# TeamOfProfGuo/Few_Shot_Seg_CWT

Measured on AMD Instinct MI355X. Metric: episodes/sec (473x473, 1-shot, R50) at 1/2/4/8 MI355X; mIoU vs ref, higher is better.
Workload: dtype fp32 (conv stack at fp32 width on the bf16 MFMA: every fp32 operand split exactly into bf16 hi + mid + lo, the six products >= 2^-24 |a||b| summed in fp32; inner loop, CWT, classifier fp32); 1 GPU; CWT inference episode (validate_transformer, batch_size_val=1): PASCAL split-0 1-shot ResNet-50 PSPNet 473x473, adapt_iter 200, heads 4; image_size=473, shot=1, layers=50

## Files before the change

### few_shot_seg_cwt_amd/csrc/conv_body.h

```cpp
#pragma once
#include "common.h"
#include "kernels.h"

namespace cwt {

typedef __bf16 bf16x8 __attribute__((ext_vector_type(8)));

#define CWT_LDS __attribute__((address_space(3)))
#define CWT_GLB __attribute__((address_space(1)))

__device__ __forceinline__ void glds16(const void* src, char* lds_dst) {
  __builtin_amdgcn_global_load_lds((const CWT_GLB void*)src, (CWT_LDS void*)lds_dst, 16, 0, 0);
}

template <int N>
__device__ __forceinline__ void wait_vmcnt() {
  asm volatile("s_waitcnt vmcnt(%0)" ::"n"(N) : "memory");
}

template <int LPT>
__device__ __forceinline__ void wait_tiles(int n) {
  if (n <= 0)
    wait_vmcnt<0>();
  else if (n == 1)
    wait_vmcnt<LPT>();
  else if (n == 2)
    wait_vmcnt<2 * LPT>();
  else if (n == 3)
    wait_vmcnt<3 * LPT>();
  else if (n == 4)
    wait_vmcnt<4 * LPT>();
  else
    wait_vmcnt<5 * LPT>();
}

__device__ __forceinline__ void block_sync_lds() {
  asm volatile("s_waitcnt lgkmcnt(0)" ::: "memory");
  __builtin_amdgcn_s_barrier();
  asm volatile("" ::: "memory");
}

struct Res8 {
  f32x4 a, b;
};
template <int PREC>
__device__ __forceinline__ Res8 load_res8(const ConvSArgs& a, int m, int co) {
  Res8 r;
  if (a.res) {
    const f32x4* rp = (const f32x4*)(a.res + (long)m * a.res_ld + co);
    r.a = rp[0];
    r.b = rp[1];
  } else if (a.res_s) {
    if (PREC == 1) {
      r.a = *(const f32x4*)(a.res_s + (long)m * a.Co + co);
      r.b = f32x4{0.f, 0.f, 0.f, 0.f};
    } else {
      const __bf16* rp = a.res_s + ((long)m * (a.Co >> 5) + (co >> 5)) * 64 + (co & 31);
      r.a = *(const f32x4*)rp;
      r.b = *(const f32x4*)(rp + 32);
    }
  } else {
    r.a = r.b = f32x4{0.f, 0.f, 0.f, 0.f};
  }
  return r;
}

template <int PREC>
__device__ __forceinline__ void store_out8(const ConvSArgs& a, int m, int co, const float* v, const float* sc,
                                           const float* sh, const Res8& rs) {
  float o[8];
#pragma unroll
  for (int i = 0; i < 8; ++i) o[i] = fmaf(v[i], sc[i], sh[i]);
  if (a.res) {
#pragma unroll
    for (int i = 0; i < 4; ++i) {
      o[i] += rs.a[i];
      o[4 + i] += rs.b[i];
    }
  } else if (a.res_s) {
    const bf16x8 rh = __builtin_bit_cast(bf16x8, rs.a), rl = __builtin_bit_cast(bf16x8, rs.b);
#pragma unroll
    for (int i = 0; i < 8; ++i) o[i] += PREC == 1 ? (float)rh[i] : (float)rh[i] + (float)rl[i];
  }
  if (a.relu) {
#pragma unroll
    for (int i = 0; i < 8; ++i) o[i] = fmaxf(o[i], 0.f);
  }
  if (a.y) {
    f32x4* yp = (f32x4*)(a.y + (long)m * a.y_ld + a.y_off + co);
    yp[0] = f32x4{o[0], o[1], o[2], o[3]};
    yp[1] = f32x4{o[4], o[5], o[6], o[7]};
  }
  if (a.ys) {
    bf16x8 hi, lo;
#pragma unroll
    for (int i = 0; i < 8; ++i) {
      hi[i] = (__bf16)o[i];
      lo[i] = (__bf16)(o[i] - (float)hi[i]);
    }
    if (PREC == 1) {
      *(bf16x8*)(a.ys + (long)m * a.Co + co) = hi;
    } else {
      __bf16* sp = a.ys + ((long)m * (a.Co >> 5) + (co >> 5)) * 64 + (co & 31);
      *(bf16x8*)sp = hi;
      *(bf16x8*)(sp + 32) = lo;
    }
  }
}

__device__ __forceinline__ void split3_bf16(const f32x4& x0, const f32x4& x1, bf16x8& h, bf16x8& m, bf16x8& l) {
#pragma unroll
  for (int i = 0; i < 8; ++i) {
    const float v = i < 4 ? x0[i] : x1[i - 4];
    const __bf16 hv = (__bf16)v;
    const float r = v - (float)hv;
    const __bf16 mv = (__bf16)r;
    h[i] = hv;
    m[i] = mv;
    l[i] = (__bf16)(r - (float)mv);
  }
}

template <int BM, int BN, int WAVES_M, int WAVES_N, int NSTG, int PREC, int PF>
__device__ __forceinline__ void conv_s_body(const ConvSArgs& a) {
  static_assert(PREC == 0 || PREC == 1 || PREC == 3 || PREC == 6,
                "PREC: 3 = bf16x3 over the S-layout, 1 = plain bf16, 0 = exact fp32 (f32 MFMA), "
                "6 = fp32 operands split three ways in registers (bf16x6)");
  constexpr int NW = WAVES_M * WAVES_N;
  constexpr int WM = BM / WAVES_M, WN = BN / WAVES_N;
  constexpr int FM = WM / 16, FN = WN / 16;
  constexpr int LA = BM / (8 * NW), LB = BN / (8 * NW);
  constexpr int NLO = PREC == 6 ? BN / 16 : 0;
  constexpr int LBL = PREC == 6 ? (NLO + NW - 1) / NW : 0;
  constexpr int LPT = LA + LB + LBL;
  constexpr int LO_OFF = (BM + BN) * 128;
  constexpr int STG_BYTES = (BM + BN) * 128 + (PREC == 6 ? BN * 64 : 0);
  static_assert(LA * 8 * NW == BM && LB * 8 * NW == BN, "tile rows must split into 8-row pieces per wave");
  static_assert(NSTG >= 2 && NSTG <= 6, "ring depth");
  constexpr int EP_ROWS = WM < 32 ? WM : 32;
  constexpr int EP_LD = WN + 4;
  constexpr int EP_BYTES = NW * EP_ROWS * EP_LD * 4;
  constexpr int SMEM = NSTG * STG_BYTES > EP_BYTES ? NSTG * STG_BYTES : EP_BYTES;
  __shared__ __attribute__((aligned(16))) char smem[SMEM];

  const int tid = threadIdx.x;
  const int lane = tid & 63;
  const int wv = __builtin_amdgcn_readfirstlane(tid >> 6);
  const int wm = wv / WAVES_N, wn = wv % WAVES_N;
  int mt, nt, ks;
  conv_tile_coords(mt, nt, ks);
  const bool batched = PREC == 6 && a.batch > 1;
  const int bidx = batched ? ks : 0;
  if (batched) ks = 0;
  const char* xs_b = (const char*)a.xs + (batched ? bidx * a.xs_bstride : 0L);
  const __bf16* ws_b = a.ws + (batched ? bidx * a.ws_bstride : 0L);
  const __bf16* wl_b = a.ws_lo + (batched ? bidx * a.wl_bstride : 0L);
  float* part_b = a.part + (batched ? (long)bidx * a.M * a.Co : 0L);
  const int m0 = mt * BM, n0 = nt * BN;
  const int kt_begin = ks * a.kt_per_split;
  const int kt_end = min(a.ktiles, kt_begin + a.kt_per_split);
  const int T = kt_end - kt_begin;
  if constexpr ((PF & 64) != 0) {
    asm volatile("" ::"s"(T));
    return;
  }


  const int lrow = lane >> 3, lslot = lane & 7;
  const int cblocks = a.Ci >> (PREC == 1 ? 6 : 5);
  int a_ih0[LA], a_iw0[LA], a_pix0[LA], a_ch[LA];
  const int HoWo = a.Ho * a.Wo;
#pragma unroll
  for (int j = 0; j < LA; ++j) {
    const int r = (wv * LA + j) * 8 + lrow;
    a_ch[j] = (lslot ^ ((r >> 1) & 7)) * 8;
    const int m = m0 + r;
    if (m < a.M) {
      const int n = m / HoWo;
      const int rem = m - n * HoWo;
      const int oh = rem / a.Wo;
      const int ow = rem - oh * a.Wo;
      a_ih0[j] = oh * a.stride - a.pad;
      a_iw0[j] = ow * a.stride - a.pad;
      a_pix0[j] = (n * a.Hi + a_ih0[j]) * a.Wi + a_iw0[j];
    } else {
      a_ih0[j] = -(1 << 28);
      a_iw0[j] = 0;
      a_pix0[j] = 0;
    }
  }
  const int b_rowlen = a.ktiles_total * 64;
  int b_off[LB];
#pragma unroll
  for (int j = 0; j < LB; ++j) {
    const int r = (wv * LB + j) * 8 + lrow;
    b_off[j] = (n0 + r) * b_rowlen + (lslot ^ ((r >> 1) & 7)) * 8;
  }

  int i_cb, i_ky, i_kx;
  {
    const int taps = a.kh * a.kw;
    i_cb = kt_begin / taps;
    const int tap = kt_begin - i_cb * taps;
    i_ky = tap / a.kw;
    i_kx = tap - i_ky * a.kw;
  }
  int i_kt = kt_begin;
  constexpr bool DUAL = (PF & 128) != 0;
  static_assert(!DUAL || (PREC == 6 && (PF & 8) != 0), "dual A source: x6 with buffer addressing");
  __amdgpu_buffer_rsrc_t rsA, rsB, rsL, rsA2;
  int a_roff[LA], b_voff[LB], l_voff[LBL > 0 ? LBL : 1], a_roff2[DUAL ? LA : 1];
#if defined(__HIP_DEVICE_COMPILE__)
  if constexpr (DUAL) {
    const int cbl2 = a.Ci2 >> 5;
    rsA2 = __builtin_amdgcn_make_buffer_rsrc((void*)a.xs2, (short)0, (int)((long)a.N * a.Hi2 * a.Wi2 * cbl2 * 128),
                                             0x00020000);
#pragma unroll
    for (int j = 0; j < LA; ++j) {
      const int m = m0 + (wv * LA + j) * 8 + lrow;
      const int n = m / HoWo, rem = m - n * HoWo;
      const int oh = rem / a.Wo, ow = rem - oh * a.Wo;
      const int pix2 = (n * a.Hi2 + oh * a.stride2) * a.Wi2 + ow * a.stride2;
      a_roff2[j] = m < a.M ? (pix2 * cbl2 * 64 + a_ch[j]) * 2 : (int)0x80000000;
    }
  }
  if constexpr ((PF & 8) != 0) {
    const int cbl = a.Ci >> (PREC == 1 ? 6 : 5);
    const long a_bytes = (long)a.N * a.Hi * a.Wi * cbl * 128;
    rsA = __builtin_amdgcn_make_buffer_rsrc((void*)xs_b, (short)0, (int)a_bytes, 0x00020000);
    rsB = __builtin_amdgcn_make_buffer_rsrc((void*)ws_b, (short)0, (int)((long)a.Co * a.ktiles_total * 128), 0x00020000);
#pragma unroll
    for (int j = 0; j < LA; ++j) a_roff[j] = (a_pix0[j] * cbl * 64 + a_ch[j]) * 2;
#pragma unroll
    for (int j = 0; j < LB; ++j) b_voff[j] = b_off[j] * 2;
    if constexpr (PREC == 6) {
      rsL = __builtin_amdgcn_make_buffer_rsrc((void*)wl_b, (short)0, (int)((long)a.Co * a.ktiles_total * 64),
                                              0x00020000);
#pragma unroll
      for (int j = 0; j < LBL; ++j) {
        const int q = (wv * LBL + j) % NLO;
        const int r = q * 16 + (lane >> 2);
        l_voff[j] = (n0 + r) * a.ktiles_total * 64 + (((lane & 3) ^ ((r >> 2) & 3)) << 4);
      }
    }
  }
#endif
  auto issue = [&](int stg) {
    if (PF & 4) return;
    char* sb = smem + stg * STG_BYTES;
#if defined(__HIP_DEVICE_COMPILE__)
    if constexpr ((PF & 8) != 0) {
      const int dy = i_ky * a.dil, dx = i_kx * a.dil;
      const int uni = ((dy * a.Wi + dx) * cblocks + i_cb) * 128;
      bool second = false;
      if constexpr (DUAL) {
        second = i_kt >= a.kt_switch;
        if (second) {
          const unsigned uni2 = (unsigned)(i_kt - a.kt_switch) * 128u;
#pragma unroll
          for (int j = 0; j < LA; ++j)
            __builtin_amdgcn_raw_ptr_buffer_load_lds(rsA2, (CWT_LDS void*)(sb + (wv * LA + j) * 1024), 16,
                                                     (int)((unsigned)a_roff2[j] + uni2), 0, 0, 0);
        }
      }
      if (!second) {
#pragma unroll
        for (int j = 0; j < LA; ++j) {
          const int ih = a_ih0[j] + dy, iw = a_iw0[j] + dx;
          const bool in = (unsigned)ih < (unsigned)a.Hi && (unsigned)iw < (unsigned)a.Wi;
          __builtin_amdgcn_raw_ptr_buffer_load_lds(rsA, (CWT_LDS void*)(sb + (wv * LA + j) * 1024), 16,
                                                   in ? a_roff[j] + uni : (int)0x80000000, 0, 0, 0);
        }
      }
#pragma unroll
      for (int j = 0; j < LB; ++j)
        __builtin_amdgcn_raw_ptr_buffer_load_lds(rsB, (CWT_LDS void*)(sb + BM * 128 + (wv * LB + j) * 1024), 16,
                                                 b_voff[j], i_kt * 128, 0, 0);
      if constexpr (PREC == 6) {
#pragma unroll
        for (int j = 0; j < LBL; ++j)
          __builtin_amdgcn_raw_ptr_buffer_load_lds(rsL, (CWT_LDS void*)(sb + LO_OFF + ((wv * LBL + j) % NLO) * 1024), 16,
                                                   l_voff[j], i_kt * 64, 0, 0);
      }
      ++i_kt;
      if (++i_kx == a.kw) {
        i_kx = 0;
        if (++i_ky == a.kh) {
          i_ky = 0;
          ++i_cb;
        }
      }
      return;
    }
#endif
    const int dy = i_ky * a.dil, dx = i_kx * a.dil;
    const int shift = dy * a.Wi + dx;
#pragma unroll
    for (int j = 0; j < LA; ++j) {
      const int ih = a_ih0[j] + dy, iw = a_iw0[j] + dx;
      const bool in = (unsigned)ih < (unsigned)a.Hi && (unsigned)iw < (unsigned)a.Wi;
      const __bf16* src = in ? a.xs + ((a_pix0[j] + shift) * cblocks + i_cb) * 64 + a_ch[j] : a.zero;
      glds16(src, sb + (wv * LA + j) * 1024);
    }
#pragma unroll
    for (int j = 0; j < LB; ++j) glds16(a.ws + b_off[j] + i_kt * 64, sb + BM * 128 + (wv * LB + j) * 1024);
    ++i_kt;
    if (++i_kx == a.kw) {
      i_kx = 0;
      if (++i_ky == a.kh) {
        i_ky = 0;
        ++i_cb;
      }
    }
  };

  f32x4 acc[FM][FN];
#pragma unroll
  for (int i = 0; i < FM; ++i)
#pragma unroll
    for (int j = 0; j < FN; ++j) acc[i][j] = f32x4{0.f, 0.f, 0.f, 0.f};

  const int fr = lane & 15, fk = lane >> 4;
  const int swz = (fr >> 1) & 7;
  const int off_hi = fr * 128 + ((fk ^ swz) << 4);
  const int off_lo = fr * 128 + (((4 + fk) ^ swz) << 4);
  const int off_a0 = PREC == 6 ? fr * 128 + (((2 * fk) ^ swz) << 4) : off_hi;
  const int off_a1 = PREC == 6 ? fr * 128 + (((2 * fk + 1) ^ swz) << 4) : off_lo;
  const int off_l = fr * 64 + ((fk ^ ((fr >> 2) & 3)) << 4);
  const int a_row0 = wm * WM, b_row0 = BM + wn * WN;

  constexpr bool LAZY_B = PREC == 6 && (PF & 3) == 0 && FN >= 8;
  struct Frags {
    bf16x8 ah[FM], al[FM], bh[LAZY_B ? 1 : FN], bl[LAZY_B ? 1 : FN];
    bf16x8 bo[PREC == 6 && !LAZY_B ? FN : 1];
  };
  auto read_frags = [&](Frags& F, int stg) {
    const char* sb = smem + stg * STG_BYTES;
#pragma unroll
    for (int j = 0; j < (LAZY_B ? 0 : FN); ++j) {
      const char* p = sb + (b_row0 + j * 16) * 128;
      F.bh[j] = *(const bf16x8*)(p + off_hi);
      F.bl[j] = *(const bf16x8*)(p + off_lo);
    }
#pragma unroll
    for (int i = 0; i < FM; ++i) {
      const char* p = sb + (a_row0 + i * 16) * 128;
      F.ah[i] = *(const bf16x8*)(p + off_a0);
      F.al[i] = *(const bf16x8*)(p + off_a1);
    }
    if constexpr (PREC == 6 && !LAZY_B) {
#pragma unroll
      for (int j = 0; j < FN; ++j) F.bo[j] = *(const bf16x8*)(sb + LO_OFF + (wn * WN + j * 16) * 64 + off_l);
    }
  };
  auto mfmas = [&](const Frags& F, int stg) {
    if (PF & 2) {
#pragma unroll
      for (int i = 0; i < FM; ++i) asm volatile("" ::"v"(F.ah[i]), "v"(F.al[i]));
#pragma unroll
      for (int j = 0; j < (LAZY_B ? 1 : FN); ++j)
        asm volatile("" ::"v"(F.bh[j]), "v"(F.bl[j]), "v"(F.bo[j < (PREC == 6 && !LAZY_B ? FN : 1) ? j : 0]));
      return;
    }
    if constexpr (LAZY_B) {
      const char* sb = smem + stg * STG_BYTES;
      bf16x8 as[FM][3];
#pragma unroll
      for (int i = 0; i < FM; ++i)
        if constexpr ((PF & 16) != 0) {
          as[i][0] = F.ah[i];
          as[i][1] = F.al[i];
          as[i][2] = F.ah[i];
        } else {
          split3_bf16(__builtin_bit_cast(f32x4, F.ah[i]), __builtin_bit_cast(f32x4, F.al[i]), as[i][0], as[i][1],
                      as[i][2]);
        }
#pragma unroll
      for (int j = 0; j < FN; ++j) {
        const char* p = sb + (b_row0 + j * 16) * 128;
        const bf16x8 bh = *(const bf16x8*)(p + off_hi), bm = *(const bf16x8*)(p + off_lo);
        const bf16x8 bl = *(const bf16x8*)(sb + LO_OFF + (wn * WN + j * 16) * 64 + off_l);
#pragma unroll
        for (int i = 0; i < FM; ++i) {
          acc[i][j] = __builtin_amdgcn_mfma_f32_16x16x32_bf16(as[i][1], bm, acc[i][j], 0, 0, 0);
          acc[i][j] = __builtin_amdgcn_mfma_f32_16x16x32_bf16(as[i][2], bh, acc[i][j], 0, 0, 0);
          acc[i][j] = __builtin_amdgcn_mfma_f32_16x16x32_bf16(as[i][0], bl, acc[i][j], 0, 0, 0);
          acc[i][j] = __builtin_amdgcn_mfma_f32_16x16x32_bf16(as[i][1], bh, acc[i][j], 0, 0, 0);
          acc[i][j] = __builtin_amdgcn_mfma_f32_16x16x32_bf16(as[i][0], bm, acc[i][j], 0, 0, 0);
          acc[i][j] = __builtin_amdgcn_mfma_f32_16x16x32_bf16(as[i][0], bh, acc[i][j], 0, 0, 0);
        }
      }
    } else if constexpr (PREC == 6) {
#pragma unroll
      for (int i = 0; i < FM; ++i) {
        bf16x8 ah, am, al;
        split3_bf16(__builtin_bit_cast(f32x4, F.ah[i]), __builtin_bit_cast(f32x4, F.al[i]), ah, am, al);
#pragma unroll
        for (int j = 0; j < FN; ++j) {
          acc[i][j] = __builtin_amdgcn_mfma_f32_16x16x32_bf16(am, F.bl[j], acc[i][j], 0, 0, 0);
          acc[i][j] = __builtin_amdgcn_mfma_f32_16x16x32_bf16(al, F.bh[j], acc[i][j], 0, 0, 0);
          acc[i][j] = __builtin_amdgcn_mfma_f32_16x16x32_bf16(ah, F.bo[j], acc[i][j], 0, 0, 0);
          acc[i][j] = __builtin_amdgcn_mfma_f32_16x16x32_bf16(am, F.bh[j], acc[i][j], 0, 0, 0);
          acc[i][j] = __builtin_amdgcn_mfma_f32_16x16x32_bf16(ah, F.bl[j], acc[i][j], 0, 0, 0);
          acc[i][j] = __builtin_amdgcn_mfma_f32_16x16x32_bf16(ah, F.bh[j], acc[i][j], 0, 0, 0);
        }
      }
    } else {
#pragma unroll
    for (int i = 0; i < FM; ++i)
#pragma unroll
      for (int j = 0; j < FN; ++j) {
        if (PREC == 0) {
          const f32x4 a0 = __builtin_bit_cast(f32x4, F.ah[i]), a1 = __builtin_bit_cast(f32x4, F.al[i]);
          const f32x4 b0 = __builtin_bit_cast(f32x4, F.bh[j]), b1 = __builtin_bit_cast(f32x4, F.bl[j]);
#pragma unroll
          for (int s = 0; s < 4; ++s) acc[i][j] = __builtin_amdgcn_mfma_f32_16x16x4f32(a0[s], b0[s], acc[i][j], 0, 0, 0);
#pragma unroll
          for (int s = 0; s < 4; ++s) acc[i][j] = __builtin_amdgcn_mfma_f32_16x16x4f32(a1[s], b1[s], acc[i][j], 0, 0, 0);
        } else if (PREC == 1) {
          acc[i][j] = __builtin_amdgcn_mfma_f32_16x16x32_bf16(F.ah[i], F.bh[j], acc[i][j], 0, 0, 0);
          acc[i][j] = __builtin_amdgcn_mfma_f32_16x16x32_bf16(F.al[i], F.bl[j], acc[i][j], 0, 0, 0);
        } else {
          acc[i][j] = __builtin_amdgcn_mfma_f32_16x16x32_bf16(F.al[i], F.bh[j], acc[i][j], 0, 0, 0);
          acc[i][j] = __builtin_amdgcn_mfma_f32_16x16x32_bf16(F.ah[i], F.bl[j], acc[i][j], 0, 0, 0);
          acc[i][j] = __builtin_amdgcn_mfma_f32_16x16x32_bf16(F.ah[i], F.bh[j], acc[i][j], 0, 0, 0);
        }
      }
    }
  };

  if constexpr ((PF & 1) == 0) {
#pragma unroll
    for (int s = 0; s < NSTG - 1; ++s)
      if (s < T) issue(s);

    for (int t = 0; t < T; ++t) {
      wait_tiles<LPT>(min(NSTG - 2, T - 1 - t));
      block_sync_lds();
      if (t + NSTG - 1 < T) issue((t + NSTG - 1) % NSTG);
      Frags F;
      read_frags(F, t % NSTG);
      mfmas(F, t % NSTG);
    }
  } else {
#pragma unroll
    for (int s = 0; s < NSTG; ++s)
      if (s < T) issue(s);
    Frags F0, F1;
    if (T > 0) {
      wait_tiles<LPT>(min(NSTG - 1, T - 1));
      block_sync_lds();
      read_frags(F0, 0);
    }
    auto step = [&](int t, Frags& cur, Frags& nxt) {
      if (t + 1 < T) {
        wait_tiles<LPT>(min(T - t - 2, NSTG - 2));
        block_sync_lds();
        if (t + NSTG < T) issue(t % NSTG);
        read_frags(nxt, (t + 1) % NSTG);
      }
      mfmas(cur, -1);
    };
    for (int t = 0; t < T; t += 2) {
      step(t, F0, F1);
      if (t + 1 < T) step(t + 1, F1, F0);
    }
  }

  wait_vmcnt<0>();
  if constexpr ((PF & 32) != 0) {
#pragma unroll
    for (int i = 0; i < FM; ++i)
#pragma unroll
      for (int j = 0; j < FN; ++j) asm volatile("" ::"v"(acc[i][j]));
    return;
  }
  block_sync_lds();
  float* ep = (float*)smem + wv * (EP_ROWS * EP_LD);
  constexpr int LPR = WN / 8;
  constexpr int RPR = 64 / LPR;
  static_assert(LPR * 8 == WN && RPR * LPR == 64 && EP_ROWS % RPR == 0, "epilogue geometry");
  const int er = lane / LPR, eg = lane - er * LPR;
  const int co = n0 + wn * WN + eg * 8;
  float sc[8], sh[8];
#pragma unroll
  for (int i = 0; i < 8; ++i) {
    sc[i] = a.part ? 1.f : a.scale[co + i];
    sh[i] = a.part ? 0.f : a.shift[co + i];
  }
  const int fq = lane >> 4;
  constexpr int NPASS = WM / EP_ROWS, RR = EP_ROWS / RPR;
  const int mrow = m0 + wm * WM + er;
  Res8 resb[2][RR];
  const bool fused = !a.part;
#pragma unroll
  for (int rr = 0; rr < RR; ++rr)
    if (fused) resb[0][rr] = load_res8<PREC>(a, min(mrow + rr * RPR, a.M - 1), co);
#pragma unroll
  for (int pass = 0; pass < NPASS; ++pass) {
#pragma unroll
    for (int fi = 0; fi < EP_ROWS / 16; ++fi)
#pragma unroll
      for (int j = 0; j < FN; ++j)
#pragma unroll
        for (int q = 0; q < 4; ++q) ep[(fi * 16 + fq * 4 + q) * EP_LD + j * 16 + fr] = acc[pass * (EP_ROWS / 16) + fi][j][q];
    asm volatile("s_waitcnt lgkmcnt(0)" ::: "memory");
    f32x4 v0[RR], v1[RR];
#pragma unroll
    for (int rr = 0; rr < RR; ++rr) {
      const int r = rr * RPR + er;
      v0[rr] = *(const f32x4*)(ep + r * EP_LD + eg * 8);
      v1[rr] = *(const f32x4*)(ep + r * EP_LD + eg * 8 + 4);
    }
    if (pass + 1 < NPASS && fused) {
#pragma unroll
      for (int rr = 0; rr < RR; ++rr)
        resb[(pass + 1) & 1][rr] = load_res8<PREC>(a, min(mrow + (pass + 1) * EP_ROWS + rr * RPR, a.M - 1), co);
    }
#pragma unroll
    for (int rr = 0; rr < RR; ++rr) {
      const int m = mrow + pass * EP_ROWS + rr * RPR;
      if (m < a.M) {
        if (!fused) {
          f32x4* pp = (f32x4*)(part_b + ((long)ks * a.M + m) * a.Co + co);
          pp[0] = v0[rr];
          pp[1] = v1[rr];
        } else {
          const float v[8] = {v0[rr][0], v0[rr][1], v0[rr][2], v0[rr][3], v1[rr][0], v1[rr][1], v1[rr][2], v1[rr][3]};
          store_out8<PREC>(a, m, co, v, sc, sh, resb[pass & 1][rr]);
        }
      }
    }
    asm volatile("s_waitcnt lgkmcnt(0)" ::: "memory");
  }
}

ConvPlan plan_heuristic_s(int M, int Co, int ktiles);
void launch_tiles_x6(int stage, const ConvSArgs& a, const ConvPlan& p, dim3 grid, hipStream_t st);
}
```

### few_shot_seg_cwt_amd/csrc/conv_forms.h

```cpp
#pragma once
#include <type_traits>

#include "kernels.h"

namespace cwt {

#define CWT_CONV_FORMS(X, A)                                                                   \
  X(256, 256, 0, 2, 4, 2, 0, 0) A(256, 256, 1, 0) A(256, 256, 2, 0)                            \
  X(256, 128, 0, 4, 2, 3, 0, 0) X(256, 128, 1, 4, 2, 3, 1, 0) A(256, 128, 2, 1)                \
  X(128, 256, 0, 2, 4, 3, 0, 0) X(128, 256, 1, 2, 4, 3, 1, 0) A(128, 256, 2, 1)                \
  X(128, 128, 0, 2, 2, 3, 0, 0) X(128, 128, 1, 2, 2, 3, 1, 0) X(128, 128, 2, 2, 4, 3, 1, 0)    \
  X(128, 128, 4, 2, 2, 2, 0, 0)                                                                \
  X(128, 64, 0, 2, 2, 3, 0, 0) X(128, 64, 1, 2, 2, 3, 1, 0) X(128, 64, 2, 4, 2, 3, 1, 0)       \
  X(64, 128, 0, 2, 2, 3, 0, 0) X(64, 128, 1, 2, 2, 3, 1, 0) X(64, 128, 2, 2, 4, 3, 1, 0)       \
  X(64, 64, 0, 2, 2, 4, 0, 0) X(64, 64, 1, 2, 2, 4, 1, 0) X(64, 64, 2, 2, 4, 4, 1, 0)          \
         \
  X(64, 64, 8, 2, 2, 4, 2, 1) X(64, 64, 9, 2, 2, 4, 4, 1)                                      \
                                             \
  X(128, 128, 10, 2, 4, 3, 3, 1) X(128, 128, 11, 2, 4, 3, 5, 1)

#define CWT_CONV_FORMS_X6(X, A)                                                                \
  X(256, 256, 3, 4, 2, 2, 0, 0) X(256, 128, 3, 8, 1, 2, 0, 0) X(128, 256, 3, 4, 2, 2, 0, 0)    \
  X(128, 128, 3, 4, 1, 3, 0, 0) X(128, 128, 5, 4, 1, 2, 0, 0)                                  \
  X(128, 64, 3, 4, 1, 3, 0, 0) X(128, 64, 5, 4, 1, 2, 0, 0)                                    \
  X(64, 128, 3, 4, 1, 3, 0, 0) X(64, 128, 5, 4, 1, 2, 0, 0)                                    \
  X(64, 64, 3, 4, 1, 4, 0, 0)                                                                  \
    \
      \
                                           \
  X(128, 128, 12, 4, 1, 2, 16, 0) X(128, 128, 14, 4, 1, 2, 4, 0) X(128, 128, 15, 4, 1, 2, 2, 0) \
  X(128, 128, 16, 4, 1, 2, 6, 0) X(128, 128, 17, 4, 1, 2, 38, 0) X(128, 128, 18, 4, 1, 2, 64, 0) \
                                                \
  X(256, 256, 13, 4, 2, 2, 16, 0)                                                              \
    \
    \
  X(128, 128, 24, 2, 2, 2, 128, 0) X(128, 128, 25, 4, 1, 2, 128, 0)                            \
  X(128, 64, 25, 4, 1, 2, 128, 0) X(64, 128, 25, 4, 1, 2, 128, 0)

constexpr int kConvDualVar = 20;

struct ConvForm {
  int bm, bn, var, waves_m, waves_n, nstg, pf;
  bool fixed_tile;
  int alias;
};
const ConvForm* find_conv_form(int prec, int bm, int bn, int var);
const ConvForm* fixed_tile_form(int prec, int var);

template <int LAST, class F>
void with_stage(int stage, F&& f) {
  if constexpr (LAST > 0)
    if (stage >= 0 && stage < LAST) return with_stage<LAST - 1>(stage, f);
  f(std::integral_constant<int, LAST>{});
}

template <class Fam, int STAGE>
void launch_form(const ConvPlan& p, const ConvSArgs& a, dim3 grid, hipStream_t st) {
#define CWT_ROW(BM, BN, VAR, WM, WN, NS, PF, FIXED)     \
  if (p.bm == BM && p.bn == BN && p.var == VAR)         \
    return Fam::template launch<BM, BN, WM, WN, NS, (FIXED && Fam::kStudyStage0) ? 0 : STAGE, PF>(a, grid, st);
#define CWT_ALIAS(BM, BN, VAR, TARGET)
  CWT_CONV_FORMS(CWT_ROW, CWT_ALIAS)
  if constexpr (Fam::kX6) {
    CWT_CONV_FORMS_X6(CWT_ROW, CWT_ALIAS)
  }
#undef CWT_ROW
#undef CWT_ALIAS
}

#define CWT_CONV_FAMILY(NAME, KERNEL, X6, STUDY_STAGE0)                                        \
  struct NAME {                                                                                \
    static constexpr bool kX6 = X6, kStudyStage0 = STUDY_STAGE0;                               \
    template <int BM, int BN, int WM, int WN, int NS, int STAGE, int PF>                       \
    static void launch(const ConvSArgs& a, dim3 grid, hipStream_t st) {                        \
      hipLaunchKernelGGL((KERNEL<BM, BN, WM, WN, NS, STAGE, PF>), grid, dim3(WM * WN * 64), 0, st, a); \
    }                                                                                          \
  }

}
```

### few_shot_seg_cwt_amd/csrc/conv_x6.hip

```cpp
#include "conv_body.h"
#include "conv_forms.h"

namespace cwt {

template <int BM, int BN, int WAVES_M, int WAVES_N, int NSTG, int STAGE, int PF = 0>
__global__ __launch_bounds__(WAVES_M* WAVES_N * 64) void conv_igemm_x6(ConvSArgs a) {
  constexpr int STG = (BM + BN) * 128 + BN * 64;
  constexpr int NS = NSTG * STG <= 163840 ? NSTG : 163840 / STG;
  static_assert(NS >= 2, "x6: a two-stage ring must fit in LDS");
  conv_s_body<BM, BN, WAVES_M, WAVES_N, NS, 6, (PF | 8)>(a);
}

__global__ void split_w3_kernel(const float* w, long n8, int K, __bf16* ws, __bf16* wl) {
  const long idx = (long)blockIdx.x * blockDim.x + threadIdx.x;
  if (idx >= n8) return;
  const long e = idx * 8;
  const long r = e / K;
  const int k = (int)(e - r * K);
  const f32x4 v0 = *(const f32x4*)(w + e), v1 = *(const f32x4*)(w + e + 4);
  bf16x8 h, m, l;
  split3_bf16(v0, v1, h, m, l);
  __bf16* sp = ws + (r * (K >> 5) + (k >> 5)) * 64 + (k & 31);
  *(bf16x8*)sp = h;
  *(bf16x8*)(sp + 32) = m;
  *(bf16x8*)(wl + (r * (K >> 5) + (k >> 5)) * 32 + (k & 31)) = l;
}

int launch_split_w3(const float* w, long R, int K, __bf16* ws, __bf16* wl, hipStream_t st) {
  if (K % 32) return fail(CWT_EARG, "split_w3: K % 32");
  const long n8 = R * K / 8;
  hipLaunchKernelGGL(split_w3_kernel, dim3((unsigned)((n8 + 255) / 256)), dim3(256), 0, st, w, n8, K, ws, wl);
  CWT_LAUNCH_CHECK();
  return 0;
}

__global__ __launch_bounds__(1024) void occupy_kernel(long ticks) {
  extern __shared__ char occ_lds[];
  const unsigned long long t0 = __builtin_amdgcn_s_memrealtime();
  if (threadIdx.x == 0) occ_lds[0] = 0;
  while (__builtin_amdgcn_s_memrealtime() - t0 < (unsigned long long)ticks) __builtin_amdgcn_s_sleep(127);
}

int launch_occupy(int nwg, int us, hipStream_t st) {
  constexpr int kLds = 160 * 1024;
  static const hipError_t attr =
      hipFuncSetAttribute((const void*)occupy_kernel, hipFuncAttributeMaxDynamicSharedMemorySize, kLds);
  if (attr != hipSuccess) return fail(CWT_ESTATE, "occupy: 160 KB of dynamic LDS refused");
  hipLaunchKernelGGL(occupy_kernel, dim3(nwg), dim3(1024), kLds, st, (long)us * 100);
  CWT_LAUNCH_CHECK();
  return 0;
}

CWT_CONV_FAMILY(FamX6, conv_igemm_x6, true, false);

void launch_tiles_x6(int stage, const ConvSArgs& a, const ConvPlan& p, dim3 grid, hipStream_t st) {
  with_stage<8>(stage, [&](auto s) { launch_form<FamX6, decltype(s)::value>(p, a, grid, st); });
}

}
```

Measured before the change: 403.6 episodes/s.

## Add GEMM-shaped load path for 1x1 unpadded x6 convolutions

Adds a specialized x6 conv body variant for 1x1, pad-0 convolutions. It precomputes pixel offsets once and issues buffer loads with a per-tile soffset, instead of recomputing tap/bounds addressing for each k-tile. It also lets waves whose M rows are entirely out of range skip fragment reads, MFMAs and the epilogue while still joining the ring barriers. This removes per-tile address arithmetic and wasted work on tail tiles, at the cost of more template instantiations and a new getenv-controlled path that needs exact bounds handling.

```diff
diff --git a/few_shot_seg_cwt_amd/csrc/conv_body.h b/few_shot_seg_cwt_amd/csrc/conv_body.h
--- a/few_shot_seg_cwt_amd/csrc/conv_body.h
+++ b/few_shot_seg_cwt_amd/csrc/conv_body.h
@@ -168,14 +168,26 @@
 
   const int lrow = lane >> 3, lslot = lane & 7;
   const int cblocks = a.Ci >> (PREC == 1 ? 6 : 5);
+  constexpr bool GEMM = (PF & 256) != 0;
+  static_assert(!GEMM || (PREC == 6 && (PF & 8) != 0), "GEMM-shaped path: x6 with buffer addressing");
   int a_ih0[LA], a_iw0[LA], a_pix0[LA], a_ch[LA];
   const int HoWo = a.Ho * a.Wo;
+  auto gemm_pix = [&](int m, int H, int W, int stride) {
+    if (stride == 1 && W == a.Wo && H == a.Ho) return m;
+    const int n = m / HoWo, rem = m - n * HoWo;
+    const int oh = rem / a.Wo, ow = rem - oh * a.Wo;
+    return (n * H + oh * stride) * W + ow * stride;
+  };
+  const bool idle = GEMM && WAVES_N == 1 && m0 + wm * WM >= a.M;
 #pragma unroll
   for (int j = 0; j < LA; ++j) {
     const int r = (wv * LA + j) * 8 + lrow;
     a_ch[j] = (lslot ^ ((r >> 1) & 7)) * 8;
     const int m = m0 + r;
-    if (m < a.M) {
+    if constexpr (GEMM) {
+      a_pix0[j] = m < a.M ? gemm_pix(m, a.Hi, a.Wi, a.stride) : -1;
+      a_ih0[j] = a_iw0[j] = 0;
+    } else if (m < a.M) {
       const int n = m / HoWo;
       const int rem = m - n * HoWo;
       const int oh = rem / a.Wo;
@@ -218,9 +230,14 @@
 #pragma unroll
     for (int j = 0; j < LA; ++j) {
       const int m = m0 + (wv * LA + j) * 8 + lrow;
-      const int n = m / HoWo, rem = m - n * HoWo;
-      const int oh = rem / a.Wo, ow = rem - oh * a.Wo;
-      const int pix2 = (n * a.Hi2 + oh * a.stride2) * a.Wi2 + ow * a.stride2;
+      int pix2;
+      if constexpr (GEMM) {
+        pix2 = gemm_pix(m, a.Hi2, a.Wi2, a.stride2);
+      } else {
+        const int n = m / HoWo, rem = m - n * HoWo;
+        const int oh = rem / a.Wo, ow = rem - oh * a.Wo;
+        pix2 = (n * a.Hi2 + oh * a.stride2) * a.Wi2 + ow * a.stride2;
+      }
       a_roff2[j] = m < a.M ? (pix2 * cbl2 * 64 + a_ch[j]) * 2 : (int)0x80000000;
     }
   }
@@ -230,7 +247,8 @@
     rsA = __builtin_amdgcn_make_buffer_rsrc((void*)xs_b, (short)0, (int)a_bytes, 0x00020000);
     rsB = __builtin_amdgcn_make_buffer_rsrc((void*)ws_b, (short)0, (int)((long)a.Co * a.ktiles_total * 128), 0x00020000);
 #pragma unroll
-    for (int j = 0; j < LA; ++j) a_roff[j] = (a_pix0[j] * cbl * 64 + a_ch[j]) * 2;
+    for (int j = 0; j < LA; ++j)
+      a_roff[j] = GEMM && a_pix0[j] < 0 ? (int)0x80000000 : (a_pix0[j] * cbl * 64 + a_ch[j]) * 2;
 #pragma unroll
     for (int j = 0; j < LB; ++j) b_voff[j] = b_off[j] * 2;
     if constexpr (PREC == 6) {
@@ -249,7 +267,34 @@
     if (PF & 4) return;
     char* sb = smem + stg * STG_BYTES;
 #if defined(__HIP_DEVICE_COMPILE__)
-    if constexpr ((PF & 8) != 0) {
+    if constexpr (GEMM) {
+      bool second = false;
+      if constexpr (DUAL) {
+        second = i_kt >= a.kt_switch;
+        if (second) {
+#pragma unroll
+          for (int j = 0; j < LA; ++j)
+            __builtin_amdgcn_raw_ptr_buffer_load_lds(rsA2, (CWT_LDS void*)(sb + (wv * LA + j) * 1024), 16, a_roff2[j],
+                                                     (i_kt - a.kt_switch) * 128, 0, 0);
+        }
+      }
+      if (!second) {
+#pragma unroll
+        for (int j = 0; j < LA; ++j)
+          __builtin_amdgcn_raw_ptr_buffer_load_lds(rsA, (CWT_LDS void*)(sb + (wv * LA + j) * 1024), 16, a_roff[j],
+                                                   i_kt * 128, 0, 0);
+      }
+#pragma unroll
+      for (int j = 0; j < LB; ++j)
+        __builtin_amdgcn_raw_ptr_buffer_load_lds(rsB, (CWT_LDS void*)(sb + BM * 128 + (wv * LB + j) * 1024), 16,
+                                                 b_voff[j], i_kt * 128, 0, 0);
+#pragma unroll
+      for (int j = 0; j < LBL; ++j)
+        __builtin_amdgcn_raw_ptr_buffer_load_lds(rsL, (CWT_LDS void*)(sb + LO_OFF + ((wv * LBL + j) % NLO) * 1024), 16,
+                                                 l_voff[j], i_kt * 64, 0, 0);
+      ++i_kt;
+      return;
+    } else if constexpr ((PF & 8) != 0) {
       const int dy = i_ky * a.dil, dx = i_kx * a.dil;
       const int uni = ((dy * a.Wi + dx) * cblocks + i_cb) * 128;
       bool second = false;
@@ -429,18 +474,26 @@
     }
   };
 
+  static_assert(!GEMM || (PF & 1) == 0, "GEMM-shaped path: the forms without fragment prefetch");
   if constexpr ((PF & 1) == 0) {
 #pragma unroll
     for (int s = 0; s < NSTG - 1; ++s)
       if (s < T) issue(s);
 
-    for (int t = 0; t < T; ++t) {
+    auto ring_step = [&](int t) {
       wait_tiles<LPT>(min(NSTG - 2, T - 1 - t));
       block_sync_lds();
       if (t + NSTG - 1 < T) issue((t + NSTG - 1) % NSTG);
-      Frags F;
-      read_frags(F, t % NSTG);
-      mfmas(F, t % NSTG);
+    };
+    if (idle) {
+      for (int t = 0; t < T; ++t) ring_step(t);
+    } else {
+      for (int t = 0; t < T; ++t) {
+        ring_step(t);
+        Frags F;
+        read_frags(F, t % NSTG);
+        mfmas(F, t % NSTG);
+      }
     }
   } else {
 #pragma unroll
@@ -476,6 +529,7 @@
     return;
   }
   block_sync_lds();
+  if (idle) return;
   float* ep = (float*)smem + wv * (EP_ROWS * EP_LD);
   constexpr int LPR = WN / 8;
   constexpr int RPR = 64 / LPR;
diff --git a/few_shot_seg_cwt_amd/csrc/conv_forms.h b/few_shot_seg_cwt_amd/csrc/conv_forms.h
--- a/few_shot_seg_cwt_amd/csrc/conv_forms.h
+++ b/few_shot_seg_cwt_amd/csrc/conv_forms.h
@@ -39,6 +39,18 @@
 
 constexpr int kConvDualVar = 20;
 
+#define CWT_CONV_GEMM_ROWS_X6(G)                                                               \
+  G(128, 128, 3) G(64, 64, 3) G(128, 128, 4) G(128, 128, 5) G(128, 64, 5) G(64, 128, 5)        \
+  G(128, 128, 24) G(128, 128, 25) G(128, 64, 25) G(64, 128, 25) G(64, 64, 0)
+
+constexpr bool x6_gemm_row(int bm, int bn, int var) {
+#define CWT_G(BM, BN, VAR) \
+  if (bm == BM && bn == BN && var == VAR) return true;
+  CWT_CONV_GEMM_ROWS_X6(CWT_G)
+#undef CWT_G
+  return false;
+}
+
 struct ConvForm {
   int bm, bn, var, waves_m, waves_n, nstg, pf;
   bool fixed_tile;
@@ -55,10 +67,14 @@
 }
 
 template <class Fam, int STAGE>
-void launch_form(const ConvPlan& p, const ConvSArgs& a, dim3 grid, hipStream_t st) {
-#define CWT_ROW(BM, BN, VAR, WM, WN, NS, PF, FIXED)     \
-  if (p.bm == BM && p.bn == BN && p.var == VAR)         \
-    return Fam::template launch<BM, BN, WM, WN, NS, (FIXED && Fam::kStudyStage0) ? 0 : STAGE, PF>(a, grid, st);
+void launch_form(const ConvPlan& p, const ConvSArgs& a, dim3 grid, hipStream_t st, bool gemm = false) {
+#define CWT_ROW(BM, BN, VAR, WM, WN, NS, PF, FIXED)                                            \
+  if (p.bm == BM && p.bn == BN && p.var == VAR) {                                              \
+    constexpr int S = (FIXED && Fam::kStudyStage0) ? 0 : STAGE;                                \
+    if constexpr (Fam::kX6 && x6_gemm_row(BM, BN, VAR))                                        \
+      if (gemm) return Fam::template launch<BM, BN, WM, WN, NS, S, (PF) | 256>(a, grid, st);   \
+    return Fam::template launch<BM, BN, WM, WN, NS, S, PF>(a, grid, st);                       \
+  }
 #define CWT_ALIAS(BM, BN, VAR, TARGET)
   CWT_CONV_FORMS(CWT_ROW, CWT_ALIAS)
   if constexpr (Fam::kX6) {
diff --git a/few_shot_seg_cwt_amd/csrc/conv_x6.hip b/few_shot_seg_cwt_amd/csrc/conv_x6.hip
--- a/few_shot_seg_cwt_amd/csrc/conv_x6.hip
+++ b/few_shot_seg_cwt_amd/csrc/conv_x6.hip
@@ -53,8 +53,15 @@
 
 CWT_CONV_FAMILY(FamX6, conv_igemm_x6, true, false);
 
+static bool x6_gemm_body(const ConvSArgs& a) {
+  if (a.kh != 1 || a.kw != 1 || a.pad != 0) return false;
+  const char* v = getenv("CWT_X6_GEMM_BODY");
+  return !(v && v[0] == '0');
+}
+
 void launch_tiles_x6(int stage, const ConvSArgs& a, const ConvPlan& p, dim3 grid, hipStream_t st) {
-  with_stage<8>(stage, [&](auto s) { launch_form<FamX6, decltype(s)::value>(p, a, grid, st); });
+  const bool gemm = x6_gemm_body(a);
+  with_stage<8>(stage, [&](auto s) { launch_form<FamX6, decltype(s)::value>(p, a, grid, st, gemm); });
 }
 
 }
```

Result: faster. 409.5 episodes/s (median of 6 runs) (+1.5%).
